# jy0205/Pyramid-Flow

Hardware: NVIDIA H100
Metric: dit_step_latent_tokens_per_sec (higher is better)
Workload: dtype bf16

## Files before the change

pyramid_flow_b200/csrc/pf_common.cuh:

```cuda
#pragma once

#include <cuda.h>
#include <cuda_bf16.h>
#include <cuda_runtime.h>
#include <stdint.h>

namespace pf {

void set_error(const char* fmt, ...);
int  check_launch(const char* what);

#define PF_REQUIRE(cond, ...)                  \
  do {                                         \
    if (!(cond)) {                             \
      ::pf::set_error(__VA_ARGS__);            \
      return -1;                               \
    }                                          \
  } while (0)

int encode_tensor_map(CUtensorMap* map, CUtensorMapDataType dtype, uint32_t rank, const void* base,
                      const uint64_t* dims, const uint64_t* strides_bytes , const uint32_t* box,
                      CUtensorMapSwizzle swizzle,
                      const uint32_t* elem_strides = nullptr );

int num_sms();
int get_option(int key);
int ensure_dyn_smem(const void* kernel, int bytes, const char* what);

__device__ __forceinline__ uint32_t smem_u32(const void* p) {
  return static_cast<uint32_t>(__cvta_generic_to_shared(p));
}

__device__ __forceinline__ bool elect_one() {
  uint32_t pred = 0;
  asm volatile(
      "{\n\t"
      ".reg .b32 %%rx;\n\t"
      ".reg .pred %%px;\n\t"
      "elect.sync %%rx|%%px, 0xffffffff;\n\t"
      "selp.b32 %0, 1, 0, %%px;\n\t"
      "}\n"
      : "=r"(pred));
  return pred != 0;
}

__device__ __forceinline__ void mbar_init(uint64_t* bar, uint32_t count) {
  asm volatile("mbarrier.init.shared::cta.b64 [%0], %1;" ::"r"(smem_u32(bar)), "r"(count) : "memory");
}
__device__ __forceinline__ void fence_barrier_init() {
  asm volatile("fence.mbarrier_init.release.cluster;" ::: "memory");
}
__device__ __forceinline__ void mbar_arrive_expect_tx(uint64_t* bar, uint32_t bytes) {
  asm volatile("mbarrier.arrive.expect_tx.shared::cta.b64 _, [%0], %1;" ::"r"(smem_u32(bar)), "r"(bytes)
               : "memory");
}
__device__ __forceinline__ void mbar_arrive(uint64_t* bar) {
  asm volatile("mbarrier.arrive.shared::cta.b64 _, [%0];" ::"r"(smem_u32(bar)) : "memory");
}
__device__ __forceinline__ bool mbar_try_wait(uint64_t* bar, uint32_t parity) {
  uint32_t ok;
  asm volatile(
      "{\n\t"
      ".reg .pred p;\n\t"
      "mbarrier.try_wait.parity.shared::cta.b64 p, [%1], %2, %3;\n\t"
      "selp.b32 %0, 1, 0, p;\n\t"
      "}\n"
      : "=r"(ok)
      : "r"(smem_u32(bar)), "r"(parity), "r"(0x989680u)
      : "memory");
  return ok != 0;
}
__device__ __forceinline__ bool mbar_test(uint64_t* bar, uint32_t parity) {
  uint32_t ok;
  asm volatile(
      "{\n\t"
      ".reg .pred p;\n\t"
      "mbarrier.test_wait.parity.shared::cta.b64 p, [%1], %2;\n\t"
      "selp.b32 %0, 1, 0, p;\n\t"
      "}\n"
      : "=r"(ok)
      : "r"(smem_u32(bar)), "r"(parity)
      : "memory");
  return ok != 0;
}
__device__ __forceinline__ void mbar_wait(uint64_t* bar, uint32_t parity) {
  while (!mbar_try_wait(bar, parity)) {
  }
}

__device__ __forceinline__ void tma_prefetch_desc(const CUtensorMap* m) {
  asm volatile("prefetch.tensormap [%0];" ::"l"(reinterpret_cast<uint64_t>(m)) : "memory");
}
__device__ __forceinline__ void tma_load_2d(void* smem_dst, const CUtensorMap* m, uint64_t* bar, int c0, int c1) {
  asm volatile(
      "cp.async.bulk.tensor.2d.shared::cluster.global.mbarrier::complete_tx::bytes [%0], [%1, {%3, %4}], [%2];"
      ::"r"(smem_u32(smem_dst)), "l"(reinterpret_cast<uint64_t>(m)), "r"(smem_u32(bar)), "r"(c0), "r"(c1)
      : "memory");
}
__device__ __forceinline__ void tma_load_3d(void* smem_dst, const CUtensorMap* m, uint64_t* bar, int c0, int c1,
                                            int c2) {
  asm volatile(
      "cp.async.bulk.tensor.3d.shared::cluster.global.mbarrier::complete_tx::bytes [%0], [%1, {%3, %4, %5}], [%2];"
      ::"r"(smem_u32(smem_dst)), "l"(reinterpret_cast<uint64_t>(m)), "r"(smem_u32(bar)), "r"(c0), "r"(c1), "r"(c2)
      : "memory");
}
__device__ __forceinline__ void tma_load_4d(void* smem_dst, const CUtensorMap* m, uint64_t* bar, int c0, int c1,
                                            int c2, int c3) {
  asm volatile(
      "cp.async.bulk.tensor.4d.shared::cluster.global.mbarrier::complete_tx::bytes [%0], [%1, {%3, %4, %5, %6}], "
      "[%2];" ::"r"(smem_u32(smem_dst)),
      "l"(reinterpret_cast<uint64_t>(m)), "r"(smem_u32(bar)), "r"(c0), "r"(c1), "r"(c2), "r"(c3)
      : "memory");
}
__device__ __forceinline__ void tma_load_5d(void* smem_dst, const CUtensorMap* m, uint64_t* bar, int c0, int c1,
                                            int c2, int c3, int c4) {
  asm volatile(
      "cp.async.bulk.tensor.5d.shared::cluster.global.mbarrier::complete_tx::bytes [%0], [%1, {%3, %4, %5, %6, "
      "%7}], [%2];" ::"r"(smem_u32(smem_dst)),
      "l"(reinterpret_cast<uint64_t>(m)), "r"(smem_u32(bar)), "r"(c0), "r"(c1), "r"(c2), "r"(c3), "r"(c4)
      : "memory");
}
__device__ __forceinline__ void fence_proxy_async_smem() {
  asm volatile("fence.proxy.async.shared::cta;" ::: "memory");
}

__device__ __forceinline__ void wgmma_fence() { asm volatile("wgmma.fence.sync.aligned;" ::: "memory"); }
__device__ __forceinline__ void wgmma_commit() { asm volatile("wgmma.commit_group.sync.aligned;" ::: "memory"); }
template <int N>
__device__ __forceinline__ void wgmma_wait() {
  asm volatile("wgmma.wait_group.sync.aligned %0;" ::"n"(N) : "memory");
}
template <int N>
__device__ __forceinline__ void wgmma_reg_fence(float (&d)[N]) {
#pragma unroll
  for (int i = 0; i < N; ++i) asm volatile("" : "+f"(d[i])::"memory");
}
template <int REGS>
__device__ __forceinline__ void setmaxnreg_inc() {
  asm volatile("setmaxnreg.inc.sync.aligned.u32 %0;" ::"n"(REGS));
}
template <int REGS>
__device__ __forceinline__ void setmaxnreg_dec() {
  asm volatile("setmaxnreg.dec.sync.aligned.u32 %0;" ::"n"(REGS));
}
__device__ __forceinline__ void named_bar_sync(int id, int threads) {
  asm volatile("bar.sync %0, %1;" ::"r"(id), "r"(threads) : "memory");
}

__device__ __forceinline__ void wgmma_ss_n128(float (&d)[64], uint64_t desc_a, uint64_t desc_b, uint32_t accumulate) {
  asm volatile(
      "{\n\t"
      ".reg .pred p;\n\t"
      "setp.ne.b32 p, %66, 0;\n\t"
      "wgmma.mma_async.sync.aligned.m64n128k16.f32.bf16.bf16 "
      "{%0, %1, %2, %3, %4, %5, %6, %7, %8, %9, %10, %11, %12, %13, %14, %15, %16, %17, %18, %19, %20, %21, %22, %23, %24, %25, %26, %27, %28, %29, %30, %31, %32, %33, %34, %35, %36, %37, %38, %39, %40, %41, %42, %43, %44, %45, %46, %47, %48, %49, %50, %51, %52, %53, %54, %55, %56, %57, %58, %59, %60, %61, %62, %63}, %64, %65, p, 1, 1, 0, 0;\n\t"
      "}\n"
      : "+f"(d[0]), "+f"(d[1]), "+f"(d[2]), "+f"(d[3]), "+f"(d[4]), "+f"(d[5]), "+f"(d[6]), "+f"(d[7]), "+f"(d[8]), "+f"(d[9]), "+f"(d[10]), "+f"(d[11]), "+f"(d[12]), "+f"(d[13]), "+f"(d[14]), "+f"(d[15]), "+f"(d[16]), "+f"(d[17]), "+f"(d[18]), "+f"(d[19]), "+f"(d[20]), "+f"(d[21]), "+f"(d[22]), "+f"(d[23]), "+f"(d[24]), "+f"(d[25]), "+f"(d[26]), "+f"(d[27]), "+f"(d[28]), "+f"(d[29]), "+f"(d[30]), "+f"(d[31]), "+f"(d[32]), "+f"(d[33]), "+f"(d[34]), "+f"(d[35]), "+f"(d[36]), "+f"(d[37]), "+f"(d[38]), "+f"(d[39]), "+f"(d[40]), "+f"(d[41]), "+f"(d[42]), "+f"(d[43]), "+f"(d[44]), "+f"(d[45]), "+f"(d[46]), "+f"(d[47]), "+f"(d[48]), "+f"(d[49]), "+f"(d[50]), "+f"(d[51]), "+f"(d[52]), "+f"(d[53]), "+f"(d[54]), "+f"(d[55]), "+f"(d[56]), "+f"(d[57]), "+f"(d[58]), "+f"(d[59]), "+f"(d[60]), "+f"(d[61]), "+f"(d[62]), "+f"(d[63])
      : "l"(desc_a), "l"(desc_b), "r"(accumulate)
      : "memory");
}
__device__ __forceinline__ void wgmma_ss_n64(float (&d)[32], uint64_t desc_a, uint64_t desc_b, uint32_t accumulate) {
  asm volatile(
      "{\n\t"
      ".reg .pred p;\n\t"
      "setp.ne.b32 p, %34, 0;\n\t"
      "wgmma.mma_async.sync.aligned.m64n64k16.f32.bf16.bf16 "
      "{%0, %1, %2, %3, %4, %5, %6, %7, %8, %9, %10, %11, %12, %13, %14, %15, %16, %17, %18, %19, %20, %21, %22, %23, %24, %25, %26, %27, %28, %29, %30, %31}, %32, %33, p, 1, 1, 0, 0;\n\t"
      "}\n"
      : "+f"(d[0]), "+f"(d[1]), "+f"(d[2]), "+f"(d[3]), "+f"(d[4]), "+f"(d[5]), "+f"(d[6]), "+f"(d[7]), "+f"(d[8]), "+f"(d[9]), "+f"(d[10]), "+f"(d[11]), "+f"(d[12]), "+f"(d[13]), "+f"(d[14]), "+f"(d[15]), "+f"(d[16]), "+f"(d[17]), "+f"(d[18]), "+f"(d[19]), "+f"(d[20]), "+f"(d[21]), "+f"(d[22]), "+f"(d[23]), "+f"(d[24]), "+f"(d[25]), "+f"(d[26]), "+f"(d[27]), "+f"(d[28]), "+f"(d[29]), "+f"(d[30]), "+f"(d[31])
      : "l"(desc_a), "l"(desc_b), "r"(accumulate)
      : "memory");
}
__device__ __forceinline__ void wgmma_rs_n64_tb(float (&d)[32], const uint32_t (&a)[4], uint64_t desc_b) {
  asm volatile(
      "{\n\t"
      ".reg .pred p;\n\t"
      "setp.ne.b32 p, 1, 0;\n\t"
      "wgmma.mma_async.sync.aligned.m64n64k16.f32.bf16.bf16 "
      "{%0, %1, %2, %3, %4, %5, %6, %7, %8, %9, %10, %11, %12, %13, %14, %15, %16, %17, %18, %19, %20, %21, %22, %23, %24, %25, %26, %27, %28, %29, %30, %31}, {%32, %33, %34, %35}, %36, p, 1, 1, 1;\n\t"
      "}\n"
      : "+f"(d[0]), "+f"(d[1]), "+f"(d[2]), "+f"(d[3]), "+f"(d[4]), "+f"(d[5]), "+f"(d[6]), "+f"(d[7]), "+f"(d[8]), "+f"(d[9]), "+f"(d[10]), "+f"(d[11]), "+f"(d[12]), "+f"(d[13]), "+f"(d[14]), "+f"(d[15]), "+f"(d[16]), "+f"(d[17]), "+f"(d[18]), "+f"(d[19]), "+f"(d[20]), "+f"(d[21]), "+f"(d[22]), "+f"(d[23]), "+f"(d[24]), "+f"(d[25]), "+f"(d[26]), "+f"(d[27]), "+f"(d[28]), "+f"(d[29]), "+f"(d[30]), "+f"(d[31])
      : "r"(a[0]), "r"(a[1]), "r"(a[2]), "r"(a[3]), "l"(desc_b)
      : "memory");
}
template <int BN>
__device__ __forceinline__ void wgmma_ss(float (&d)[BN / 2], uint64_t desc_a, uint64_t desc_b, uint32_t accumulate) {
  static_assert(BN == 128 || BN == 64, "wgmma_ss: tile widths 128 and 64 are instantiated");
  if constexpr (BN == 128) wgmma_ss_n128(d, desc_a, desc_b, accumulate);
  else wgmma_ss_n64(d, desc_a, desc_b, accumulate);
}

__device__ __forceinline__ uint64_t make_smem_desc(uint32_t saddr, uint32_t lbo_bytes, uint32_t sbo_bytes) {
  uint64_t d = 0;
  d |= static_cast<uint64_t>((saddr & 0x3FFFFu) >> 4);
  d |= static_cast<uint64_t>((lbo_bytes >> 4) & 0x3FFFu) << 16;
  d |= static_cast<uint64_t>((sbo_bytes >> 4) & 0x3FFFu) << 32;
  d |= static_cast<uint64_t>(1) << 62;
  return d;
}
__device__ __forceinline__ uint64_t make_smem_desc_kmajor_sw128(uint32_t saddr) {
  return make_smem_desc(saddr, 16, 1024);
}

constexpr int PIPE_THREADS = 384;
constexpr int PIPE_CONSUMER_WARPS = 8;
constexpr int PIPE_BM = 128;
constexpr int PIPE_BK = 64;
template <int BN>
struct PipeCfg {
  static constexpr int A_BYTES = PIPE_BM * PIPE_BK * 2;
  static constexpr int B_BYTES = BN * PIPE_BK * 2;
  static constexpr int STAGE_BYTES = A_BYTES + B_BYTES;
  static constexpr int STAGES = (BN >= 128) ? 4 : 6;
  static constexpr int ACC_PITCH = BN + 8;
  static constexpr int ACC_BYTES = PIPE_BM * ACC_PITCH * 4;
  static constexpr int SMEM_BYTES = STAGES * STAGE_BYTES + ACC_BYTES + 1024;
};

template <int BN>
__device__ __forceinline__ void pipe_consume_tile(float (&acc)[BN / 2], uint8_t* smem, uint64_t* full_bar, uint64_t* empty_bar,
                                                  int num_kb, int wg, int& stage, uint32_t& phase) {
  using Cfg = PipeCfg<BN>;
  const int lane = threadIdx.x & 31;
  int prev = -1;
  for (int kb = 0; kb < num_kb; ++kb) {
    mbar_wait(&full_bar[stage], phase);
    const uint32_t sa = smem_u32(smem + stage * Cfg::STAGE_BYTES);
    const uint64_t da = make_smem_desc_kmajor_sw128(sa + wg * (64 * 128));
    const uint64_t db = make_smem_desc_kmajor_sw128(sa + Cfg::A_BYTES);
    wgmma_reg_fence(acc);
    wgmma_fence();
#pragma unroll
    for (int kk = 0; kk < PIPE_BK / 16; ++kk) wgmma_ss<BN>(acc, da + 2 * kk, db + 2 * kk, (kb | kk) != 0 ? 1u : 0u);
    wgmma_commit();
    wgmma_wait<1>();
    if (prev >= 0 && lane == 0) mbar_arrive(&empty_bar[prev]);
    prev = stage;
    if (++stage == Cfg::STAGES) {
      stage = 0;
      phase ^= 1;
    }
  }
  wgmma_wait<0>();
  wgmma_reg_fence(acc);
  if (prev >= 0 && lane == 0) mbar_arrive(&empty_bar[prev]);
}

template <int BN>
__device__ __forceinline__ void pipe_stage_acc(const float (&acc)[BN / 2], float* acc_tile, int wg) {
  const int w = (threadIdx.x >> 5) & 3, lane = threadIdx.x & 31;
  float* r0 = acc_tile + (wg * 64 + w * 16 + (lane >> 2)) * PipeCfg<BN>::ACC_PITCH + 2 * (lane & 3);
  float* r1 = r0 + 8 * PipeCfg<BN>::ACC_PITCH;
#pragma unroll
  for (int i = 0; i < BN / 8; ++i) {
    *reinterpret_cast<float2*>(r0 + 8 * i) = make_float2(acc[4 * i + 0], acc[4 * i + 1]);
    *reinterpret_cast<float2*>(r1 + 8 * i) = make_float2(acc[4 * i + 2], acc[4 * i + 3]);
  }
}

__device__ __forceinline__ uint32_t pack_bf16x2(float lo, float hi) {
  __nv_bfloat162 v = __floats2bfloat162_rn(lo, hi);
  return *reinterpret_cast<uint32_t*>(&v);
}
__device__ __forceinline__ float rcp_approx_f(float x) {
  float y;
  asm("rcp.approx.ftz.f32 %0, %1;" : "=f"(y) : "f"(x));
  return y;
}
__device__ __forceinline__ float ex2_approx_f(float x) {
  float y;
  asm("ex2.approx.ftz.f32 %0, %1;" : "=f"(y) : "f"(x));
  return y;
}
__device__ __forceinline__ float gelu_tanh_f(float x) {
  const float c0 = -2.0f * 0.7978845608028654f * 1.4426950408889634f;
  const float c1 = c0 * 0.044715f;
  const float x2 = x * x;
  const float nu = x * fmaf(x2, c1, c0);
  return x * rcp_approx_f(1.0f + ex2_approx_f(nu));
}
__device__ __forceinline__ float silu_f(float x) {
  return x * rcp_approx_f(1.0f + ex2_approx_f(-1.4426950408889634f * x));
}

}
```

pyramid_flow_b200/csrc/pf_gemm.cu:

```cuda
#include <cstdlib>

#include "../../include/pf_b200.h"
#include "pf_common.cuh"

namespace pf {

struct GemmArgs {
  int batches, row_begin, row_count;
  int n, k;
  int m_tiles, n_tiles;
  const float* bias;
  void* out;
  long long ldo;
  int out_batch_rows, out_row_begin, out_col_begin;
  const float* gate;
  long long gate_batch_stride;
  __nv_bfloat16* q_out;
  __nv_bfloat16* k_out;
  __nv_bfloat16* v_out;
  const float* rope;
  const float* q_norm_w;
  const float* k_norm_w;
  float norm_eps;
  int heads, head_dim, seq_len;
  int n_split;
  __nv_bfloat16* peer_qkv[PF_MAX_PEERS];
  int peer_count, peer_heads, peer_seq, peer_row0;
  int epi_staged;
};

constexpr int BM = PIPE_BM;
constexpr int BK = PIPE_BK;

__device__ __forceinline__ void store_bf16x32(__nv_bfloat16* dst, const float (&x)[32]) {
  uint4* d4 = reinterpret_cast<uint4*>(dst);
#pragma unroll
  for (int i = 0; i < 4; ++i) {
    uint4 u;
    u.x = pack_bf16x2(x[8 * i + 0], x[8 * i + 1]);
    u.y = pack_bf16x2(x[8 * i + 2], x[8 * i + 3]);
    u.z = pack_bf16x2(x[8 * i + 4], x[8 * i + 5]);
    u.w = pack_bf16x2(x[8 * i + 6], x[8 * i + 7]);
    d4[i] = u;
  }
}

__device__ __forceinline__ void load_bias32(float (&x)[32], const float* srow, const float* bias) {
  const float4* s4 = reinterpret_cast<const float4*>(srow);
#pragma unroll
  for (int i = 0; i < 8; ++i) {
    const float4 v = s4[i];
    float4 b = make_float4(0.f, 0.f, 0.f, 0.f);
    if (bias != nullptr) b = __ldg(reinterpret_cast<const float4*>(bias) + i);
    x[4 * i + 0] = v.x + b.x;
    x[4 * i + 1] = v.y + b.y;
    x[4 * i + 2] = v.z + b.z;
    x[4 * i + 3] = v.w + b.w;
  }
}

__device__ __forceinline__ void qkv_head_epilogue(const GemmArgs& g, const float* srow, int n0, int b, int pos, bool valid) {
  float x[64];
  {
    float lo[32], hi[32];
    load_bias32(lo, srow, g.bias ? g.bias + n0 : nullptr);
    load_bias32(hi, srow + 32, g.bias ? g.bias + n0 + 32 : nullptr);
#pragma unroll
    for (int i = 0; i < 32; ++i) {
      x[i] = lo[i];
      x[32 + i] = hi[i];
    }
  }
  const int inner = g.heads * g.head_dim;
  const int section = n0 / inner;
  const int head = (n0 - section * inner) / g.head_dim;
  __nv_bfloat16* base = section == 0 ? g.q_out : (section == 1 ? g.k_out : g.v_out);
  if (section < 2) {
    float s0 = 0.f, s1 = 0.f, s2 = 0.f, s3 = 0.f;
#pragma unroll
    for (int i = 0; i < 64; i += 4) {
      s0 = fmaf(x[i + 0], x[i + 0], s0);
      s1 = fmaf(x[i + 1], x[i + 1], s1);
      s2 = fmaf(x[i + 2], x[i + 2], s2);
      s3 = fmaf(x[i + 3], x[i + 3], s3);
    }
    const float ss = (s0 + s1) + (s2 + s3);
    const float r = rsqrtf(ss * (1.0f / 64.0f) + g.norm_eps);
    const float4* w4 = reinterpret_cast<const float4*>(section == 0 ? g.q_norm_w : g.k_norm_w);
#pragma unroll
    for (int i = 0; i < 16; ++i) {
      const float4 w = __ldg(w4 + i);
      x[4 * i + 0] *= r * w.x;
      x[4 * i + 1] *= r * w.y;
      x[4 * i + 2] *= r * w.z;
      x[4 * i + 3] *= r * w.w;
    }
    if (g.rope != nullptr && valid) {
      const float4* cs4 = reinterpret_cast<const float4*>(g.rope + static_cast<size_t>(pos) * 64);
#pragma unroll
      for (int i = 0; i < 16; ++i) {
        const float4 cs = __ldg(cs4 + i);
        const float a0 = x[4 * i + 0], a1 = x[4 * i + 1], a2 = x[4 * i + 2], a3 = x[4 * i + 3];
        x[4 * i + 0] = cs.x * a0 - cs.y * a1;
        x[4 * i + 1] = cs.y * a0 + cs.x * a1;
        x[4 * i + 2] = cs.z * a2 - cs.w * a3;
        x[4 * i + 3] = cs.w * a2 + cs.z * a3;
      }
    }
  }
  if (valid) {
    __nv_bfloat16* dst;
    if (g.peer_count > 1) {
      const int r = head / g.peer_heads, hl = head - r * g.peer_heads;
      dst = g.peer_qkv[r] + ((static_cast<size_t>(section) * g.peer_heads + hl) * g.peer_seq + g.peer_row0 + pos) * 64;
    } else {
      dst = base + ((static_cast<size_t>(b) * g.heads + head) * g.seq_len + pos) * 64;
    }
    float lo[32], hi[32];
#pragma unroll
    for (int i = 0; i < 32; ++i) {
      lo[i] = x[i];
      hi[i] = x[32 + i];
    }
    store_bf16x32(dst, lo);
    store_bf16x32(dst + 32, hi);
  }
}

template <int BN, int EPI>
__device__ __forceinline__ void epilogue_tile(const GemmArgs& g, const float* acc_rows, int tid, int b, int m_base, int n_base) {
  constexpr int PITCH = PipeCfg<BN>::ACC_PITCH;
  const int row = tid & 63, half = tid >> 6;
  const int m = m_base + row;
  const bool valid = m < g.row_count;
  const size_t out_row = static_cast<size_t>(b) * g.out_batch_rows + g.out_row_begin + m;
  const float* srow = acc_rows + row * PITCH;
  bool qkv_tile = (EPI == PF_EPI_QKV_ROPE);
  if (EPI == PF_EPI_QKV_GELU) qkv_tile = n_base < g.n_split;

  if (qkv_tile) {
    const int pos = g.out_row_begin + m;
#pragma unroll 1
    for (int h = half; h < BN / 64; h += 2) qkv_head_epilogue(g, srow + h * 64, n_base + h * 64, b, pos, valid);
  } else if (EPI == PF_EPI_GATE_RESID && g.epi_staged) {
    constexpr int VEC_PER_ROW = BN / 4, ROWS_PER_IT = 32 / VEC_PER_ROW;
    const int warp = tid >> 5, lane = tid & 31;
    const int c4 = lane % VEC_PER_ROW, rsub = lane / VEC_PER_ROW;
    const float4 gg = __ldg(reinterpret_cast<const float4*>(g.gate + b * g.gate_batch_stride + n_base) + c4);
    float4 bb = make_float4(0.f, 0.f, 0.f, 0.f);
    if (g.bias != nullptr) bb = __ldg(reinterpret_cast<const float4*>(g.bias + n_base) + c4);
    float* obase = reinterpret_cast<float*>(g.out) + g.out_col_begin + n_base + 4 * c4;
    const size_t row0 = static_cast<size_t>(b) * g.out_batch_rows + g.out_row_begin + m_base;
#pragma unroll 4
    for (int it = 0; it < 16 / ROWS_PER_IT; ++it) {
      const int rr = warp * 16 + it * ROWS_PER_IT + rsub;
      if (m_base + rr < g.row_count) {
        const float4 a4 = *reinterpret_cast<const float4*>(acc_rows + rr * PITCH + 4 * c4);
        float4* dst = reinterpret_cast<float4*>(obase + (row0 + rr) * g.ldo);
        float4 r4 = *dst;
        r4.x += gg.x * (a4.x + bb.x);
        r4.y += gg.y * (a4.y + bb.y);
        r4.z += gg.z * (a4.z + bb.z);
        r4.w += gg.w * (a4.w + bb.w);
        *dst = r4;
      }
    }
  } else {
#pragma unroll 1
    for (int c = half; c < BN / 32; c += 2) {
      const int n0 = n_base + c * 32;
      float x[32];
      load_bias32(x, srow + c * 32, g.bias ? g.bias + n0 : nullptr);
      if (EPI == PF_EPI_GELU_BF16 || EPI == PF_EPI_QKV_GELU) {
#pragma unroll
        for (int i = 0; i < 32; ++i) x[i] = gelu_tanh_f(x[i]);
      }
      if (!valid) continue;
      if (EPI == PF_EPI_STORE_BF16 || EPI == PF_EPI_GELU_BF16 || EPI == PF_EPI_QKV_GELU) {
        const int col = (EPI == PF_EPI_QKV_GELU) ? (g.out_col_begin + n0 - g.n_split) : (g.out_col_begin + n0);
        store_bf16x32(reinterpret_cast<__nv_bfloat16*>(g.out) + out_row * g.ldo + col, x);
      } else if (EPI == PF_EPI_STORE_F32) {
        float4* d4 = reinterpret_cast<float4*>(reinterpret_cast<float*>(g.out) + out_row * g.ldo + g.out_col_begin + n0);
#pragma unroll
        for (int i = 0; i < 8; ++i) d4[i] = make_float4(x[4 * i], x[4 * i + 1], x[4 * i + 2], x[4 * i + 3]);
      } else if (EPI == PF_EPI_GATE_RESID) {
        float4* d4 = reinterpret_cast<float4*>(reinterpret_cast<float*>(g.out) + out_row * g.ldo + g.out_col_begin + n0);
        const float4* g4 = reinterpret_cast<const float4*>(g.gate + b * g.gate_batch_stride + n0);
#pragma unroll
        for (int i = 0; i < 8; ++i) {
          float4 rr = d4[i];
          const float4 gg = __ldg(g4 + i);
          rr.x += gg.x * x[4 * i + 0];
          rr.y += gg.y * x[4 * i + 1];
          rr.z += gg.z * x[4 * i + 2];
          rr.w += gg.w * x[4 * i + 3];
          d4[i] = rr;
        }
      }
    }
  }
}

template <int BN, int EPI>
__global__ void __launch_bounds__(PIPE_THREADS, 1)
gemm_bf16_wgmma_kernel(const __grid_constant__ CUtensorMap tm_a, const __grid_constant__ CUtensorMap tm_b,
                       const GemmArgs g) {
  using Cfg = PipeCfg<BN>;
  constexpr int STAGES = Cfg::STAGES;
  extern __shared__ uint8_t smem_raw[];
  uint8_t* smem = reinterpret_cast<uint8_t*>((reinterpret_cast<uintptr_t>(smem_raw) + 1023) & ~uintptr_t(1023));
  float* acc_tile = reinterpret_cast<float*>(smem + STAGES * Cfg::STAGE_BYTES);

  __shared__ __align__(8) uint64_t full_bar[STAGES];
  __shared__ __align__(8) uint64_t empty_bar[STAGES];

  const int warp = threadIdx.x >> 5;
  const int wgroup = warp >> 2;

  if (threadIdx.x == 0) {
    tma_prefetch_desc(&tm_a);
    tma_prefetch_desc(&tm_b);
    for (int i = 0; i < STAGES; ++i) {
      mbar_init(&full_bar[i], 1);
      mbar_init(&empty_bar[i], PIPE_CONSUMER_WARPS);
    }
    fence_barrier_init();
  }
  __syncthreads();

  const int num_kb = (g.k + BK - 1) / BK;
  const int tiles_per_batch = g.m_tiles * g.n_tiles;
  const int total_tiles = g.batches * tiles_per_batch;

  if (wgroup == 0) {
    setmaxnreg_dec<40>();
    if (warp == 0 && elect_one()) {
      int stage = 0;
      uint32_t phase = 0;
      for (int tile = blockIdx.x; tile < total_tiles; tile += gridDim.x) {
        const int b = tile / tiles_per_batch;
        const int r = tile - b * tiles_per_batch;
        const int mt = r / g.n_tiles;
        const int nt = r - mt * g.n_tiles;
        for (int kb = 0; kb < num_kb; ++kb) {
          mbar_wait(&empty_bar[stage], phase ^ 1);
          uint8_t* sa = smem + stage * Cfg::STAGE_BYTES;
          mbar_arrive_expect_tx(&full_bar[stage], Cfg::STAGE_BYTES);
          tma_load_3d(sa, &tm_a, &full_bar[stage], kb * BK, g.row_begin + mt * BM, b);
          tma_load_2d(sa + Cfg::A_BYTES, &tm_b, &full_bar[stage], kb * BK, nt * BN);
          if (++stage == STAGES) {
            stage = 0;
            phase ^= 1;
          }
        }
      }
    }
  } else {
    setmaxnreg_inc<232>();
    const int wg = wgroup - 1;
    const int tid = threadIdx.x & 127;
    int stage = 0;
    uint32_t phase = 0;
    float acc[BN / 2];
    for (int tile = blockIdx.x; tile < total_tiles; tile += gridDim.x) {
      const int b = tile / tiles_per_batch;
      const int r = tile - b * tiles_per_batch;
      const int mt = r / g.n_tiles;
      const int nt = r - mt * g.n_tiles;
      pipe_consume_tile<BN>(acc, smem, full_bar, empty_bar, num_kb, wg, stage, phase);
      named_bar_sync(1 + wg, 128);
      pipe_stage_acc<BN>(acc, acc_tile, wg);
      named_bar_sync(1 + wg, 128);
      epilogue_tile<BN, EPI>(g, acc_tile + wg * 64 * Cfg::ACC_PITCH, tid, b, mt * BM + wg * 64, nt * BN);
    }
  }
}

template <int BN, int EPI>
static int launch_gemm(const CUtensorMap& tm_a, const CUtensorMap& tm_b, const GemmArgs& g, cudaStream_t stream) {
  using Cfg = PipeCfg<BN>;
  auto kern = gemm_bf16_wgmma_kernel<BN, EPI>;
  if (int rc = ensure_dyn_smem(reinterpret_cast<const void*>(kern), Cfg::SMEM_BYTES, "gemm")) return rc;
  const int total = g.batches * g.m_tiles * g.n_tiles;
  int grid = num_sms();
  if (grid <= 0) grid = 132;
  if (total < grid) grid = total;
  kern<<<grid, PIPE_THREADS, Cfg::SMEM_BYTES, stream>>>(tm_a, tm_b, g);
  return check_launch("pf_gemm_bf16");
}

template <int EPI>
static int dispatch_bn(int bn, const CUtensorMap& tm_a, const CUtensorMap& tm_b, const GemmArgs& g, cudaStream_t stream) {
  switch (bn) {
    case 128: return launch_gemm<128, EPI>(tm_a, tm_b, g, stream);
    case 64: return launch_gemm<64, EPI>(tm_a, tm_b, g, stream);
  }
  set_error("unsupported BLOCK_N %d", bn);
  return -1;
}

template <int EPI>
static int warm_epi() {
  int rc = ensure_dyn_smem(reinterpret_cast<const void*>(gemm_bf16_wgmma_kernel<128, EPI>), PipeCfg<128>::SMEM_BYTES, "gemm<128>");
  if (!rc) rc = ensure_dyn_smem(reinterpret_cast<const void*>(gemm_bf16_wgmma_kernel<64, EPI>), PipeCfg<64>::SMEM_BYTES, "gemm<64>");
  return rc;
}
int warmup_gemm() {
  int rc = warm_epi<PF_EPI_STORE_BF16>();
  if (!rc) rc = warm_epi<PF_EPI_GELU_BF16>();
  if (!rc) rc = warm_epi<PF_EPI_STORE_F32>();
  if (!rc) rc = warm_epi<PF_EPI_GATE_RESID>();
  if (!rc) rc = warm_epi<PF_EPI_QKV_ROPE>();
  if (!rc) rc = warm_epi<PF_EPI_QKV_GELU>();
  return rc;
}

}

extern "C" int pf_gemm_bf16(const pf_gemm_desc* d, void* stream_) {
  using namespace pf;
  cudaStream_t stream = static_cast<cudaStream_t>(stream_);
  PF_REQUIRE(d != nullptr, "pf_gemm_bf16: null descriptor");
  PF_REQUIRE(d->a && d->w, "pf_gemm_bf16: null operand");
  PF_REQUIRE(d->k > 0 && d->k % 8 == 0, "pf_gemm_bf16: k=%d must be a positive multiple of 8", d->k);
  PF_REQUIRE(d->lda % 8 == 0 && d->lda >= d->k, "pf_gemm_bf16: lda=%lld must be >= k and a multiple of 8", (long long)d->lda);
  PF_REQUIRE(d->batches > 0 && d->rows_per_batch > 0 && d->row_count > 0 && d->row_begin >= 0 &&
                 d->row_begin + d->row_count <= d->rows_per_batch,
             "pf_gemm_bf16: bad row range (batches %d rows %d begin %d count %d)", d->batches, d->rows_per_batch,
             d->row_begin, d->row_count);
  PF_REQUIRE((reinterpret_cast<uintptr_t>(d->a) & 15) == 0 && (reinterpret_cast<uintptr_t>(d->w) & 15) == 0,
             "pf_gemm_bf16: operands must be 16-byte aligned");
  const int epi = d->epilogue;
  PF_REQUIRE(epi >= 0 && epi <= PF_EPI_QKV_GELU, "pf_gemm_bf16: unknown epilogue %d", epi);

  int bn = 0;
  const bool qkv = (epi == PF_EPI_QKV_ROPE || epi == PF_EPI_QKV_GELU);
  if (qkv) {
    PF_REQUIRE(d->head_dim == 64, "pf_gemm_bf16: QKV epilogue supports head_dim 64 only (got %d)", d->head_dim);
    const int inner = d->heads * d->head_dim;
    const int nq = 3 * inner;
    PF_REQUIRE(d->q_out && d->k_out && d->v_out && d->q_norm_w && d->k_norm_w, "pf_gemm_bf16: QKV epilogue needs q/k/v outputs and norm weights");
    PF_REQUIRE(d->out_row_begin + d->row_count <= d->seq_len, "pf_gemm_bf16: QKV rows exceed seq_len");
    if (epi == PF_EPI_QKV_ROPE) {
      PF_REQUIRE(d->n == nq, "pf_gemm_bf16: QKV_ROPE needs n == 3*heads*head_dim");
    } else {
      PF_REQUIRE(d->n_split == nq && d->n > nq && d->out != nullptr, "pf_gemm_bf16: QKV_GELU needs n_split == 3*heads*head_dim < n and out");
      PF_REQUIRE(nq % 64 == 0, "pf_gemm_bf16: n_split must be a multiple of 64");
    }
  } else {
    PF_REQUIRE(d->out != nullptr, "pf_gemm_bf16: null output");
    if (epi == PF_EPI_GATE_RESID) PF_REQUIRE(d->gate != nullptr, "pf_gemm_bf16: GATE_RESID needs gate");
    const int esz = (epi == PF_EPI_STORE_F32 || epi == PF_EPI_GATE_RESID) ? 4 : 2;
    PF_REQUIRE((d->ldo * esz) % 16 == 0 && (d->out_col_begin * esz) % 16 == 0 &&
                   (reinterpret_cast<uintptr_t>(d->out) & 15) == 0,
               "pf_gemm_bf16: output must be 16-byte aligned (ldo %lld col %d)", (long long)d->ldo, d->out_col_begin);
  }
  PF_REQUIRE(d->n % 64 == 0, "pf_gemm_bf16: n=%d must be a multiple of 64", d->n);
  bn = (d->n % 128 == 0 && (epi != PF_EPI_QKV_GELU || d->n_split % 128 == 0)) ? 128 : 64;

  GemmArgs g{};
  g.batches = d->batches;
  g.row_begin = d->row_begin;
  g.row_count = d->row_count;
  g.n = d->n;
  g.k = d->k;
  g.m_tiles = (d->row_count + BM - 1) / BM;
  g.bias = d->bias;
  g.out = d->out;
  g.ldo = d->ldo;
  g.out_batch_rows = d->out_batch_rows;
  g.out_row_begin = d->out_row_begin;
  g.out_col_begin = d->out_col_begin;
  g.gate = d->gate;
  g.gate_batch_stride = d->gate_batch_stride;
  g.q_out = static_cast<__nv_bfloat16*>(d->q_out);
  g.k_out = static_cast<__nv_bfloat16*>(d->k_out);
  g.v_out = static_cast<__nv_bfloat16*>(d->v_out);
  g.rope = d->rope;
  g.q_norm_w = d->q_norm_w;
  g.k_norm_w = d->k_norm_w;
  g.norm_eps = d->norm_eps;
  g.heads = d->heads;
  g.head_dim = d->head_dim;
  g.seq_len = d->seq_len;
  g.n_split = d->n_split;
  g.epi_staged = get_option(PF_OPT_GEMM_STAGED_RESID);
  g.peer_count = d->peer_count;
  g.peer_heads = d->peer_heads;
  g.peer_seq = d->peer_seq;
  g.peer_row0 = d->peer_row0;
  for (int i = 0; i < PF_MAX_PEERS; ++i) g.peer_qkv[i] = static_cast<__nv_bfloat16*>(d->peer_qkv[i]);
  if (d->peer_count > 1) {
    PF_REQUIRE(epi == PF_EPI_QKV_ROPE && d->batches == 1, "pf_gemm_bf16: peer stores need the QKV_ROPE epilogue and batches == 1");
    PF_REQUIRE(d->peer_count <= PF_MAX_PEERS && d->peer_heads > 0 && d->peer_heads * d->peer_count >= d->heads &&
                   d->peer_row0 >= 0 && d->peer_row0 + d->out_row_begin + d->row_count <= d->peer_seq,
               "pf_gemm_bf16: bad peer layout (count %d heads/rank %d seq %d row0 %d)", d->peer_count, d->peer_heads, d->peer_seq, d->peer_row0);
    for (int i = 0; i < d->peer_count; ++i) PF_REQUIRE(d->peer_qkv[i] != nullptr, "pf_gemm_bf16: peer_qkv[%d] is null", i);
  }

  PF_REQUIRE(d->kernel_variant >= 0 && d->kernel_variant <= 2, "pf_gemm_bf16: bad kernel_variant %d", d->kernel_variant);
  PF_REQUIRE(d->kernel_variant != 1 || bn == 128, "pf_gemm_bf16: kernel_variant 1 (128-wide tiles) needs n %% 128 == 0");
  if (d->kernel_variant == 2) bn = 64;
  if (bn == 128 && d->kernel_variant == 0 && get_option(PF_OPT_GEMM_WAVE_TILING)) {
    int sms = num_sms();
    if (sms <= 0) sms = 132;
    auto cost = [&](int tile_n) -> double {
      const long long tiles = static_cast<long long>(d->batches) * ((d->row_count + BM - 1) / BM) * (d->n / tile_n);
      const long long waves = (tiles + sms - 1) / sms;
      return static_cast<double>(waves) * tile_n / (tile_n == 128 ? 1.0 : 0.75);
    };
    if (cost(64) < cost(128)) bn = 64;
  }
  CUtensorMap tm_a;
  {
    const uint64_t dims[3] = {static_cast<uint64_t>(d->k), static_cast<uint64_t>(d->rows_per_batch),
                              static_cast<uint64_t>(d->batches)};
    const uint64_t strides[2] = {static_cast<uint64_t>(d->lda) * 2,
                                 static_cast<uint64_t>(d->lda) * 2 * static_cast<uint64_t>(d->rows_per_batch)};
    const uint32_t box[3] = {BK, BM, 1};
    int rc = encode_tensor_map(&tm_a, CU_TENSOR_MAP_DATA_TYPE_BFLOAT16, 3, d->a, dims, strides, box,
                               CU_TENSOR_MAP_SWIZZLE_128B);
    if (rc) return rc;
  }

  CUtensorMap tm_b;
  {
    const uint64_t dims[2] = {static_cast<uint64_t>(d->k), static_cast<uint64_t>(d->n)};
    const uint64_t strides[1] = {static_cast<uint64_t>(d->k) * 2};
    const uint32_t box[2] = {BK, static_cast<uint32_t>(bn)};
    int rc = encode_tensor_map(&tm_b, CU_TENSOR_MAP_DATA_TYPE_BFLOAT16, 2, d->w, dims, strides, box,
                               CU_TENSOR_MAP_SWIZZLE_128B);
    if (rc) return rc;
  }
  g.n_tiles = d->n / bn;
  switch (epi) {
    case PF_EPI_STORE_BF16: return dispatch_bn<PF_EPI_STORE_BF16>(bn, tm_a, tm_b, g, stream);
    case PF_EPI_GELU_BF16: return dispatch_bn<PF_EPI_GELU_BF16>(bn, tm_a, tm_b, g, stream);
    case PF_EPI_STORE_F32: return dispatch_bn<PF_EPI_STORE_F32>(bn, tm_a, tm_b, g, stream);
    case PF_EPI_GATE_RESID: return dispatch_bn<PF_EPI_GATE_RESID>(bn, tm_a, tm_b, g, stream);
    case PF_EPI_QKV_ROPE: return dispatch_bn<PF_EPI_QKV_ROPE>(bn, tm_a, tm_b, g, stream);
    case PF_EPI_QKV_GELU: return dispatch_bn<PF_EPI_QKV_GELU>(bn, tm_a, tm_b, g, stream);
  }
  return -1;
}
```

Measured before the change: 114,300.

## Add 2-CTA cluster GEMM with 256x128 tiles and multicast B loads

Adds a new GEMM kernel that runs in 2-CTA clusters. Each CTA computes a 256x128 tile, and the weight (B) tile is split so each CTA multicasts half of it via TMA to both CTAs. Empty barriers are signalled across the cluster, and the epilogue works directly from register fragments instead of staging through shared memory. The dispatcher picks the cluster kernel by default for n%128 tiles, using a wave-cost model when wave tiling is enabled. This is meant to raise operand reuse and cut L2/HBM weight traffic, at the cost of cross-CTA synchronization, coarser tiles with worse wave quantization, and a more complex register-heavy epilogue.

```diff
diff --git a/pyramid_flow_b200/csrc/pf_common.cuh b/pyramid_flow_b200/csrc/pf_common.cuh
--- a/pyramid_flow_b200/csrc/pf_common.cuh
+++ b/pyramid_flow_b200/csrc/pf_common.cuh
@@ -123,6 +123,31 @@
 __device__ __forceinline__ void fence_proxy_async_smem() {
   asm volatile("fence.proxy.async.shared::cta;" ::: "memory");
 }
+__device__ __forceinline__ void tma_load_2d_multicast(void* smem_dst, const CUtensorMap* m, uint64_t* bar, int c0, int c1,
+                                                      uint16_t cta_mask) {
+  asm volatile(
+      "cp.async.bulk.tensor.2d.shared::cluster.global.mbarrier::complete_tx::bytes.multicast::cluster [%0], [%1, {%3, %4}], "
+      "[%2], %5;" ::"r"(smem_u32(smem_dst)),
+      "l"(reinterpret_cast<uint64_t>(m)), "r"(smem_u32(bar)), "r"(c0), "r"(c1), "h"(cta_mask)
+      : "memory");
+}
+
+__device__ __forceinline__ uint32_t cluster_ctarank() {
+  uint32_t r;
+  asm volatile("mov.u32 %0, %%cluster_ctarank;" : "=r"(r));
+  return r;
+}
+__device__ __forceinline__ void mbar_arrive_cluster(uint64_t* bar, uint32_t cta) {
+  asm volatile(
+      "{\n\t"
+      ".reg .b32 ra;\n\t"
+      "mapa.shared::cluster.u32 ra, %0, %1;\n\t"
+      "mbarrier.arrive.shared::cluster.b64 _, [ra];\n\t"
+      "}\n" ::"r"(smem_u32(bar)), "r"(cta)
+      : "memory");
+}
+__device__ __forceinline__ void cluster_arrive() { asm volatile("barrier.cluster.arrive.release.aligned;" ::: "memory"); }
+__device__ __forceinline__ void cluster_wait() { asm volatile("barrier.cluster.wait.acquire.aligned;" ::: "memory"); }
 
 __device__ __forceinline__ void wgmma_fence() { asm volatile("wgmma.fence.sync.aligned;" ::: "memory"); }
 __device__ __forceinline__ void wgmma_commit() { asm volatile("wgmma.commit_group.sync.aligned;" ::: "memory"); }
diff --git a/pyramid_flow_b200/csrc/pf_gemm.cu b/pyramid_flow_b200/csrc/pf_gemm.cu
--- a/pyramid_flow_b200/csrc/pf_gemm.cu
+++ b/pyramid_flow_b200/csrc/pf_gemm.cu
@@ -31,6 +31,10 @@
 
 constexpr int BM = PIPE_BM;
 constexpr int BK = PIPE_BK;
+
+constexpr double GEMM_RATE_CLUSTER = 1.25;
+constexpr double GEMM_RATE_128 = 1.0;
+constexpr double GEMM_RATE_64 = 0.75;
 
 __device__ __forceinline__ void store_bf16x32(__nv_bfloat16* dst, const float (&x)[32]) {
   uint4* d4 = reinterpret_cast<uint4*>(dst);
@@ -276,6 +280,261 @@
   }
 }
 
+constexpr int CBM = 256;
+constexpr int CBN = 128;
+constexpr int C_STAGES = 4;
+constexpr int C_A_BYTES = CBM * BK * 2;
+constexpr int C_B_BYTES = CBN * BK * 2;
+constexpr int C_STAGE_BYTES = C_A_BYTES + C_B_BYTES;
+constexpr int C_SMEM_BYTES = C_STAGES * C_STAGE_BYTES + 1024;
+
+__device__ __forceinline__ void cluster_consume_tile(float (&acc)[2][64], uint8_t* smem, uint64_t* full_bar, uint64_t* empty_bar,
+                                                     int num_kb, int wg, int& stage, uint32_t& phase) {
+  const int lane = threadIdx.x & 31;
+  int prev = -1;
+  for (int kb = 0; kb < num_kb; ++kb) {
+    mbar_wait(&full_bar[stage], phase);
+    const uint32_t sa = smem_u32(smem + stage * C_STAGE_BYTES);
+    const uint64_t da0 = make_smem_desc_kmajor_sw128(sa + (2 * wg + 0) * (64 * 128));
+    const uint64_t da1 = make_smem_desc_kmajor_sw128(sa + (2 * wg + 1) * (64 * 128));
+    const uint64_t db = make_smem_desc_kmajor_sw128(sa + C_A_BYTES);
+    wgmma_reg_fence(acc[0]);
+    wgmma_reg_fence(acc[1]);
+    wgmma_fence();
+#pragma unroll
+    for (int kk = 0; kk < BK / 16; ++kk) {
+      const uint32_t accum = (kb | kk) != 0 ? 1u : 0u;
+      wgmma_ss_n128(acc[0], da0 + 2 * kk, db + 2 * kk, accum);
+      wgmma_ss_n128(acc[1], da1 + 2 * kk, db + 2 * kk, accum);
+    }
+    wgmma_commit();
+    wgmma_wait<1>();
+    if (prev >= 0 && lane == 0) {
+      mbar_arrive_cluster(&empty_bar[prev], 0);
+      mbar_arrive_cluster(&empty_bar[prev], 1);
+    }
+    prev = stage;
+    if (++stage == C_STAGES) {
+      stage = 0;
+      phase ^= 1;
+    }
+  }
+  wgmma_wait<0>();
+  wgmma_reg_fence(acc[0]);
+  wgmma_reg_fence(acc[1]);
+  if (prev >= 0 && lane == 0) {
+    mbar_arrive_cluster(&empty_bar[prev], 0);
+    mbar_arrive_cluster(&empty_bar[prev], 1);
+  }
+}
+
+template <int EPI>
+__device__ __forceinline__ void epilogue_frag(const GemmArgs& g, const float (&acc)[2][64], int wg, int b, int m_base, int n_base) {
+  const int w = (threadIdx.x >> 5) & 3, lane = threadIdx.x & 31;
+  const int r_thr = wg * 128 + w * 16 + (lane >> 2);
+  const int c_thr = 2 * (lane & 3);
+  bool qkv_tile = (EPI == PF_EPI_QKV_ROPE);
+  if (EPI == PF_EPI_QKV_GELU) qkv_tile = n_base < g.n_split;
+
+  if (qkv_tile) {
+    const int inner = g.heads * g.head_dim;
+#pragma unroll
+    for (int hh = 0; hh < 2; ++hh) {
+      const int n0 = n_base + hh * 64;
+      const int section = n0 / inner;
+      const int head = (n0 - section * inner) / g.head_dim;
+      __nv_bfloat16* base = section == 0 ? g.q_out : (section == 1 ? g.k_out : g.v_out);
+      const float* nw = section == 0 ? g.q_norm_w : g.k_norm_w;
+#pragma unroll
+      for (int hr = 0; hr < 4; ++hr) {
+        const int h = hr >> 1, half = hr & 1;
+        const int m = m_base + r_thr + 64 * h + 8 * half;
+        const bool valid = m < g.row_count;
+        const int pos = g.out_row_begin + m;
+        float x[16];
+#pragma unroll
+        for (int j = 0; j < 8; ++j) {
+          float2 bb = make_float2(0.f, 0.f);
+          if (g.bias != nullptr) bb = __ldg(reinterpret_cast<const float2*>(g.bias + n0 + 8 * j + c_thr));
+          x[2 * j + 0] = acc[h][4 * (8 * hh + j) + 2 * half + 0] + bb.x;
+          x[2 * j + 1] = acc[h][4 * (8 * hh + j) + 2 * half + 1] + bb.y;
+        }
+        if (section < 2) {
+          const bool lo_first = (lane & 2) == 0;
+          float s_e[2] = {0.f, 0.f};
+#pragma unroll
+          for (int j = 0; j < 8; ++j) {
+#pragma unroll
+            for (int e = 0; e < 2; ++e) {
+              const float own = x[2 * j + e], other = __shfl_xor_sync(0xffffffffu, own, 2);
+              const float first = lo_first ? own : other, second = lo_first ? other : own;
+              s_e[e] = fmaf(first, first, s_e[e]);
+              s_e[e] = fmaf(second, second, s_e[e]);
+            }
+          }
+          const float pair = s_e[0] + s_e[1];
+          const float ss = pair + __shfl_xor_sync(0xffffffffu, pair, 1);
+          const float r = rsqrtf(ss * (1.0f / 64.0f) + g.norm_eps);
+#pragma unroll
+          for (int j = 0; j < 8; ++j) {
+            const float2 wn = __ldg(reinterpret_cast<const float2*>(nw + 8 * j + c_thr));
+            x[2 * j + 0] *= r * wn.x;
+            x[2 * j + 1] *= r * wn.y;
+          }
+          if (g.rope != nullptr && valid) {
+            const float* rp = g.rope + static_cast<size_t>(pos) * 64 + c_thr;
+#pragma unroll
+            for (int j = 0; j < 8; ++j) {
+              const float2 cs = __ldg(reinterpret_cast<const float2*>(rp + 8 * j));
+              const float a0 = x[2 * j + 0], a1 = x[2 * j + 1];
+              x[2 * j + 0] = cs.x * a0 - cs.y * a1;
+              x[2 * j + 1] = cs.y * a0 + cs.x * a1;
+            }
+          }
+        }
+        if (valid) {
+          __nv_bfloat16* dst;
+          if (g.peer_count > 1) {
+            const int pr = head / g.peer_heads, hl = head - pr * g.peer_heads;
+            dst = g.peer_qkv[pr] + ((static_cast<size_t>(section) * g.peer_heads + hl) * g.peer_seq + g.peer_row0 + pos) * 64;
+          } else {
+            dst = base + ((static_cast<size_t>(b) * g.heads + head) * g.seq_len + pos) * 64;
+          }
+#pragma unroll
+          for (int j = 0; j < 8; ++j)
+            *reinterpret_cast<uint32_t*>(dst + 8 * j + c_thr) = pack_bf16x2(x[2 * j + 0], x[2 * j + 1]);
+        }
+      }
+    }
+  } else if (EPI == PF_EPI_GATE_RESID) {
+    const float* gate = g.gate + b * g.gate_batch_stride + n_base + c_thr;
+    float* obase = reinterpret_cast<float*>(g.out) + g.out_col_begin + n_base + c_thr;
+#pragma unroll
+    for (int hr = 0; hr < 4; ++hr) {
+      const int h = hr >> 1, half = hr & 1;
+      const int m = m_base + r_thr + 64 * h + 8 * half;
+      if (m >= g.row_count) continue;
+      float2* dst = reinterpret_cast<float2*>(obase + (static_cast<size_t>(b) * g.out_batch_rows + g.out_row_begin + m) * g.ldo);
+      float2 rr[16];
+#pragma unroll
+      for (int i = 0; i < 16; ++i) rr[i] = dst[4 * i];
+#pragma unroll
+      for (int i = 0; i < 16; ++i) {
+        float2 bb = make_float2(0.f, 0.f);
+        if (g.bias != nullptr) bb = __ldg(reinterpret_cast<const float2*>(g.bias + n_base + 8 * i + c_thr));
+        const float2 gg = __ldg(reinterpret_cast<const float2*>(gate + 8 * i));
+        const float x0 = acc[h][4 * i + 2 * half + 0] + bb.x;
+        const float x1 = acc[h][4 * i + 2 * half + 1] + bb.y;
+        rr[i].x += gg.x * x0;
+        rr[i].y += gg.y * x1;
+        dst[4 * i] = rr[i];
+      }
+    }
+  } else {
+#pragma unroll
+    for (int i = 0; i < 16; ++i) {
+      const int n = n_base + 8 * i + c_thr;
+      float2 bb = make_float2(0.f, 0.f);
+      if (g.bias != nullptr) bb = __ldg(reinterpret_cast<const float2*>(g.bias + n));
+#pragma unroll
+      for (int hr = 0; hr < 4; ++hr) {
+        const int h = hr >> 1, half = hr & 1;
+        const int m = m_base + r_thr + 64 * h + 8 * half;
+        float x0 = acc[h][4 * i + 2 * half + 0] + bb.x;
+        float x1 = acc[h][4 * i + 2 * half + 1] + bb.y;
+        if (EPI == PF_EPI_GELU_BF16 || EPI == PF_EPI_QKV_GELU) {
+          x0 = gelu_tanh_f(x0);
+          x1 = gelu_tanh_f(x1);
+        }
+        if (m >= g.row_count) continue;
+        const size_t out_row = static_cast<size_t>(b) * g.out_batch_rows + g.out_row_begin + m;
+        if (EPI == PF_EPI_STORE_F32) {
+          *reinterpret_cast<float2*>(reinterpret_cast<float*>(g.out) + out_row * g.ldo + g.out_col_begin + n) = make_float2(x0, x1);
+        } else {
+          const int col = (EPI == PF_EPI_QKV_GELU) ? (g.out_col_begin + n - g.n_split) : (g.out_col_begin + n);
+          *reinterpret_cast<uint32_t*>(reinterpret_cast<__nv_bfloat16*>(g.out) + out_row * g.ldo + col) = pack_bf16x2(x0, x1);
+        }
+      }
+    }
+  }
+}
+
+template <int EPI>
+__global__ void __launch_bounds__(PIPE_THREADS, 1)
+gemm_bf16_cluster_kernel(const __grid_constant__ CUtensorMap tm_a, const __grid_constant__ CUtensorMap tm_b,
+                         const GemmArgs g) {
+  extern __shared__ uint8_t smem_raw[];
+  uint8_t* smem = reinterpret_cast<uint8_t*>((reinterpret_cast<uintptr_t>(smem_raw) + 1023) & ~uintptr_t(1023));
+
+  __shared__ __align__(8) uint64_t full_bar[C_STAGES];
+  __shared__ __align__(8) uint64_t empty_bar[C_STAGES];
+
+  const int warp = threadIdx.x >> 5;
+  const int wgroup = warp >> 2;
+  const uint32_t rank = cluster_ctarank();
+
+  if (threadIdx.x == 0) {
+    tma_prefetch_desc(&tm_a);
+    tma_prefetch_desc(&tm_b);
+    for (int i = 0; i < C_STAGES; ++i) {
+      mbar_init(&full_bar[i], 1);
+      mbar_init(&empty_bar[i], 2 * PIPE_CONSUMER_WARPS);
+    }
+    fence_barrier_init();
+  }
+  cluster_arrive();
+  cluster_wait();
+
+  const int num_kb = (g.k + BK - 1) / BK;
+  const int m_pairs = (g.m_tiles + 1) >> 1;
+  const int pairs_per_batch = m_pairs * g.n_tiles;
+  const int total_pairs = g.batches * pairs_per_batch;
+  const int cluster = blockIdx.x >> 1, clusters = gridDim.x >> 1;
+
+  if (wgroup == 0) {
+    setmaxnreg_dec<40>();
+    if (warp == 0 && elect_one()) {
+      int stage = 0;
+      uint32_t phase = 0;
+      for (int p = cluster; p < total_pairs; p += clusters) {
+        const int b = p / pairs_per_batch;
+        const int r = p - b * pairs_per_batch;
+        const int mt = 2 * (r / g.n_tiles) + static_cast<int>(rank);
+        const int nt = r % g.n_tiles;
+        for (int kb = 0; kb < num_kb; ++kb) {
+          mbar_wait(&empty_bar[stage], phase ^ 1);
+          uint8_t* sa = smem + stage * C_STAGE_BYTES;
+          mbar_arrive_expect_tx(&full_bar[stage], C_STAGE_BYTES);
+          tma_load_3d(sa, &tm_a, &full_bar[stage], kb * BK, g.row_begin + mt * CBM, b);
+          tma_load_2d_multicast(sa + C_A_BYTES + rank * (C_B_BYTES / 2), &tm_b, &full_bar[stage], kb * BK,
+                                nt * CBN + rank * (CBN / 2), 0x3);
+          if (++stage == C_STAGES) {
+            stage = 0;
+            phase ^= 1;
+          }
+        }
+      }
+    }
+    __syncwarp();
+  } else {
+    setmaxnreg_inc<232>();
+    const int wg = wgroup - 1;
+    int stage = 0;
+    uint32_t phase = 0;
+    float acc[2][64];
+    for (int p = cluster; p < total_pairs; p += clusters) {
+      const int b = p / pairs_per_batch;
+      const int r = p - b * pairs_per_batch;
+      const int mt = 2 * (r / g.n_tiles) + static_cast<int>(rank);
+      const int nt = r % g.n_tiles;
+      cluster_consume_tile(acc, smem, full_bar, empty_bar, num_kb, wg, stage, phase);
+      epilogue_frag<EPI>(g, acc, wg, b, mt * CBM, nt * CBN);
+    }
+  }
+  cluster_arrive();
+  cluster_wait();
+}
+
 template <int BN, int EPI>
 static int launch_gemm(const CUtensorMap& tm_a, const CUtensorMap& tm_b, const GemmArgs& g, cudaStream_t stream) {
   using Cfg = PipeCfg<BN>;
@@ -289,19 +548,70 @@
   return check_launch("pf_gemm_bf16");
 }
 
+static int g_cluster_slots = 0;
+
+static int cluster_slots() {
+  if (g_cluster_slots > 0) return g_cluster_slots;
+  auto kern = gemm_bf16_cluster_kernel<PF_EPI_STORE_BF16>;
+  if (int rc = ensure_dyn_smem(reinterpret_cast<const void*>(kern), C_SMEM_BYTES, "gemm cluster")) return rc;
+  cudaLaunchConfig_t cfg = {};
+  cudaLaunchAttribute attr[1];
+  attr[0].id = cudaLaunchAttributeClusterDimension;
+  attr[0].val.clusterDim.x = 2;
+  attr[0].val.clusterDim.y = 1;
+  attr[0].val.clusterDim.z = 1;
+  cfg.gridDim = dim3(2, 1, 1);
+  cfg.blockDim = dim3(PIPE_THREADS, 1, 1);
+  cfg.dynamicSmemBytes = C_SMEM_BYTES;
+  cfg.attrs = attr;
+  cfg.numAttrs = 1;
+  int n = 0;
+  if (cudaOccupancyMaxActiveClusters(&n, kern, &cfg) != cudaSuccess || n <= 0) {
+    (void)cudaGetLastError();
+    n = num_sms() > 0 ? num_sms() / 2 : 66;
+  }
+  g_cluster_slots = n;
+  return n;
+}
+
 template <int EPI>
-static int dispatch_bn(int bn, const CUtensorMap& tm_a, const CUtensorMap& tm_b, const GemmArgs& g, cudaStream_t stream) {
-  switch (bn) {
+static int launch_cluster(const CUtensorMap& tm_a, const CUtensorMap& tm_b, const GemmArgs& g, cudaStream_t stream) {
+  auto kern = gemm_bf16_cluster_kernel<EPI>;
+  if (int rc = ensure_dyn_smem(reinterpret_cast<const void*>(kern), C_SMEM_BYTES, "gemm cluster")) return rc;
+  const int slots = cluster_slots();
+  if (slots < 0) return slots;
+  const int pairs = g.batches * ((g.m_tiles + 1) / 2) * g.n_tiles;
+  cudaLaunchConfig_t cfg = {};
+  cudaLaunchAttribute attr[1];
+  attr[0].id = cudaLaunchAttributeClusterDimension;
+  attr[0].val.clusterDim.x = 2;
+  attr[0].val.clusterDim.y = 1;
+  attr[0].val.clusterDim.z = 1;
+  cfg.gridDim = dim3(2 * (pairs < slots ? pairs : slots), 1, 1);
+  cfg.blockDim = dim3(PIPE_THREADS, 1, 1);
+  cfg.dynamicSmemBytes = C_SMEM_BYTES;
+  cfg.stream = stream;
+  cfg.attrs = attr;
+  cfg.numAttrs = 1;
+  (void)cudaLaunchKernelEx(&cfg, kern, tm_a, tm_b, g);
+  return check_launch("pf_gemm_bf16");
+}
+
+template <int EPI>
+static int dispatch_tile(int tile, const CUtensorMap& tm_a, const CUtensorMap& tm_b, const GemmArgs& g, cudaStream_t stream) {
+  switch (tile) {
+    case 0: return launch_cluster<EPI>(tm_a, tm_b, g, stream);
     case 128: return launch_gemm<128, EPI>(tm_a, tm_b, g, stream);
     case 64: return launch_gemm<64, EPI>(tm_a, tm_b, g, stream);
   }
-  set_error("unsupported BLOCK_N %d", bn);
+  set_error("unsupported GEMM tile %d", tile);
   return -1;
 }
 
 template <int EPI>
 static int warm_epi() {
-  int rc = ensure_dyn_smem(reinterpret_cast<const void*>(gemm_bf16_wgmma_kernel<128, EPI>), PipeCfg<128>::SMEM_BYTES, "gemm<128>");
+  int rc = ensure_dyn_smem(reinterpret_cast<const void*>(gemm_bf16_cluster_kernel<EPI>), C_SMEM_BYTES, "gemm cluster");
+  if (!rc) rc = ensure_dyn_smem(reinterpret_cast<const void*>(gemm_bf16_wgmma_kernel<128, EPI>), PipeCfg<128>::SMEM_BYTES, "gemm<128>");
   if (!rc) rc = ensure_dyn_smem(reinterpret_cast<const void*>(gemm_bf16_wgmma_kernel<64, EPI>), PipeCfg<64>::SMEM_BYTES, "gemm<64>");
   return rc;
 }
@@ -312,6 +622,7 @@
   if (!rc) rc = warm_epi<PF_EPI_GATE_RESID>();
   if (!rc) rc = warm_epi<PF_EPI_QKV_ROPE>();
   if (!rc) rc = warm_epi<PF_EPI_QKV_GELU>();
+  if (!rc) rc = cluster_slots() > 0 ? 0 : -1;
   return rc;
 }
 
@@ -364,7 +675,6 @@
   g.row_count = d->row_count;
   g.n = d->n;
   g.k = d->k;
-  g.m_tiles = (d->row_count + BM - 1) / BM;
   g.bias = d->bias;
   g.out = d->out;
   g.ldo = d->ldo;
@@ -400,24 +710,31 @@
 
   PF_REQUIRE(d->kernel_variant >= 0 && d->kernel_variant <= 2, "pf_gemm_bf16: bad kernel_variant %d", d->kernel_variant);
   PF_REQUIRE(d->kernel_variant != 1 || bn == 128, "pf_gemm_bf16: kernel_variant 1 (128-wide tiles) needs n %% 128 == 0");
-  if (d->kernel_variant == 2) bn = 64;
-  if (bn == 128 && d->kernel_variant == 0 && get_option(PF_OPT_GEMM_WAVE_TILING)) {
+  int tile = bn == 128 ? 0 : 64;
+  if (d->kernel_variant == 2) tile = 64;
+  if (tile == 0 && d->kernel_variant == 0 && get_option(PF_OPT_GEMM_WAVE_TILING)) {
     int sms = num_sms();
     if (sms <= 0) sms = 132;
-    auto cost = [&](int tile_n) -> double {
-      const long long tiles = static_cast<long long>(d->batches) * ((d->row_count + BM - 1) / BM) * (d->n / tile_n);
-      const long long waves = (tiles + sms - 1) / sms;
-      return static_cast<double>(waves) * tile_n / (tile_n == 128 ? 1.0 : 0.75);
-    };
-    if (cost(64) < cost(128)) bn = 64;
-  }
+    const int slots = cluster_slots();
+    const long long mt128 = (d->row_count + BM - 1) / BM, mt256 = (d->row_count + CBM - 1) / CBM;
+    const long long waves0 = (d->batches * ((mt256 + 1) / 2) * (d->n / 128) + slots - 1) / (slots > 0 ? slots : 66);
+    const long long waves128 = (d->batches * mt128 * (d->n / 128) + sms - 1) / sms;
+    const long long waves64 = (d->batches * mt128 * (d->n / 64) + sms - 1) / sms;
+    const double cost0 = waves0 * 2.0 / GEMM_RATE_CLUSTER, cost128 = waves128 * 1.0 / GEMM_RATE_128,
+                 cost64 = waves64 * 0.5 / GEMM_RATE_64;
+    if (cost128 < cost0 && cost128 <= cost64) tile = 128;
+    else if (cost64 < cost0) tile = 64;
+  }
+  if (tile != 0) bn = tile;
+  const int tile_rows = tile == 0 ? CBM : BM;
+  g.m_tiles = (d->row_count + tile_rows - 1) / tile_rows;
   CUtensorMap tm_a;
   {
     const uint64_t dims[3] = {static_cast<uint64_t>(d->k), static_cast<uint64_t>(d->rows_per_batch),
                               static_cast<uint64_t>(d->batches)};
     const uint64_t strides[2] = {static_cast<uint64_t>(d->lda) * 2,
                                  static_cast<uint64_t>(d->lda) * 2 * static_cast<uint64_t>(d->rows_per_batch)};
-    const uint32_t box[3] = {BK, BM, 1};
+    const uint32_t box[3] = {BK, static_cast<uint32_t>(tile_rows), 1};
     int rc = encode_tensor_map(&tm_a, CU_TENSOR_MAP_DATA_TYPE_BFLOAT16, 3, d->a, dims, strides, box,
                                CU_TENSOR_MAP_SWIZZLE_128B);
     if (rc) return rc;
@@ -427,19 +744,19 @@
   {
     const uint64_t dims[2] = {static_cast<uint64_t>(d->k), static_cast<uint64_t>(d->n)};
     const uint64_t strides[1] = {static_cast<uint64_t>(d->k) * 2};
-    const uint32_t box[2] = {BK, static_cast<uint32_t>(bn)};
+    const uint32_t box[2] = {BK, static_cast<uint32_t>(tile == 0 ? CBN / 2 : bn)};
     int rc = encode_tensor_map(&tm_b, CU_TENSOR_MAP_DATA_TYPE_BFLOAT16, 2, d->w, dims, strides, box,
                                CU_TENSOR_MAP_SWIZZLE_128B);
     if (rc) return rc;
   }
   g.n_tiles = d->n / bn;
   switch (epi) {
-    case PF_EPI_STORE_BF16: return dispatch_bn<PF_EPI_STORE_BF16>(bn, tm_a, tm_b, g, stream);
-    case PF_EPI_GELU_BF16: return dispatch_bn<PF_EPI_GELU_BF16>(bn, tm_a, tm_b, g, stream);
-    case PF_EPI_STORE_F32: return dispatch_bn<PF_EPI_STORE_F32>(bn, tm_a, tm_b, g, stream);
-    case PF_EPI_GATE_RESID: return dispatch_bn<PF_EPI_GATE_RESID>(bn, tm_a, tm_b, g, stream);
-    case PF_EPI_QKV_ROPE: return dispatch_bn<PF_EPI_QKV_ROPE>(bn, tm_a, tm_b, g, stream);
-    case PF_EPI_QKV_GELU: return dispatch_bn<PF_EPI_QKV_GELU>(bn, tm_a, tm_b, g, stream);
+    case PF_EPI_STORE_BF16: return dispatch_tile<PF_EPI_STORE_BF16>(tile, tm_a, tm_b, g, stream);
+    case PF_EPI_GELU_BF16: return dispatch_tile<PF_EPI_GELU_BF16>(tile, tm_a, tm_b, g, stream);
+    case PF_EPI_STORE_F32: return dispatch_tile<PF_EPI_STORE_F32>(tile, tm_a, tm_b, g, stream);
+    case PF_EPI_GATE_RESID: return dispatch_tile<PF_EPI_GATE_RESID>(tile, tm_a, tm_b, g, stream);
+    case PF_EPI_QKV_ROPE: return dispatch_tile<PF_EPI_QKV_ROPE>(tile, tm_a, tm_b, g, stream);
+    case PF_EPI_QKV_GELU: return dispatch_tile<PF_EPI_QKV_GELU>(tile, tm_a, tm_b, g, stream);
   }
   return -1;
 }
```

New measurement: 127,800 (median of 6 runs). +11.9%, better.
